# Audio-WestlakeU/NBSS

Measured on AMD Instinct MI355X. Metric: utterances/sec (4 s, 6ch, 129 freqs) SpatialNet bf16 train at 1/2/4/8 MI355X, higher is better.
Workload: dtype bf16; 1 GPU; SpatialNet-small 6ch->2spk, 4-s 8-kHz utterances (32000 samples), n_fft 256/hop 128 (F=129, T=251), 8 layers, full train step (STFT..Adam), bf16 stream + fp32 master/stats, 32 utterances per GPU per step; batch_per_gpu=32, global_batch=32, parallelism=dp1

## Files before the change

### nbss_amd/csrc/full.hip

```cpp
#include <stdlib.h>
#include "launch.h"
#include "layout.h"
#include "prof.h"
#include "blocks.h"
#include "wgrad.h"
#include "fold.h"
#include "foldk.h"
#include "geom.h"
#include "side.h"

#define FL_H 96
#define FL_SQ 8
#define FL_TT_MAX 8
#define FL_KS (FL_H / 32)
#define FL_MT (FL_H / 16)
#define FL_KSF_MAX 5
#define FL_KSF_BIG 9
#define FL_THREADS 512


#define FL_TASK_LOOP_BEGIN(NTASK, WMAT)                                                                                  \
    constexpr bool TPF = TT < 8;                                                                                         \
    Frag<T> anext[KSFM];                                                                                                 \
    if (TPF && w < (NTASK)) {                                                                                            \
        _Pragma("unroll") for (int ks = 0; ks < KSFM; ++ks)                                                              \
            if (ks < ksf) wfrag_load(anext[ks], (WMAT) + (size_t)(w / mtf) * mtf * ksf * 512, w % mtf, ksf, ks);         \
    }                                                                                                                    \
    for (int task = w; task < (NTASK); task += nw) {                                                                     \
        const int ch = task / mtf, mt = task % mtf;                                                                      \
        f32x4 acc = F32X4_ZERO;                                                                                          \
        Frag<T> a[KSFM];                         \
        if (TPF) {                                                                                                       \
            _Pragma("unroll") for (int ks = 0; ks < KSFM; ++ks) a[ks] = anext[ks];                                       \
            const int nx = task + nw;                                                                                    \
            if (nx < (NTASK)) {                                                                                          \
                _Pragma("unroll") for (int ks = 0; ks < KSFM; ++ks)                                                      \
                    if (ks < ksf) wfrag_load(anext[ks], (WMAT) + (size_t)(nx / mtf) * mtf * ksf * 512, nx % mtf, ksf, ks); \
            }                                                                                                            \
        } else {                                                                                                         \
            _Pragma("unroll") for (int ks = 0; ks < KSFM; ++ks)                                                          \
                if (ks < ksf) wfrag_load(a[ks], (WMAT) + (size_t)ch * mtf * ksf * 512, mt, ksf, ks);                     \
        }                                                                                                                \
        _Pragma("unroll") for (int ks = 0; ks < KSFM; ++ks) {                                                            \
            if (ks < ksf) {                                                                                              \
                Frag<T> bq;                                                                                              \
                if (l15 < TT) frag_load(bq, s + ((size_t)ch * TT + l15) * FK + ks * 32 + 8 * g4);                        \
                else frag_zero(bq);                                                                                      \
                acc = mma(a[ks], bq, acc);                                                                               \
            }                                                                                                            \
        }
#define FL_TASK_LOOP_END }

template <class T, int KSFM, int HH, int NSQ, int TT>
__global__ __launch_bounds__(FL_THREADS, HH == 96 && TT == 8 ? 4 : 1)
void full_fwd_kernel(nbss_cfg c, const float* __restrict__ lnw, const float* __restrict__ lnb,
                                                       const float* __restrict__ bs, const float* __restrict__ bfull,
                                                       const float* __restrict__ bu, const T* __restrict__ Wsq,
                                                       const T* __restrict__ Wfull, const T* __restrict__ Wusq,
                                                       const T* __restrict__ x, T* __restrict__ y, int flip) {
    NBSS_LDS(smem);
    const int F = c.F, T_ = c.T;
    const int mtf = cdiv(F, 16), ksf = cdiv(F, 32), FK = ksf * 32, FM = mtf * 16;
    T* s = reinterpret_cast<T*>(smem);
    T* z = s + NSQ * TT * FK;
    const int ntt = cdiv(T_, TT);
    const int bid = flip_bid(flip);
    const int b = bid / ntt, t0 = (bid % ntt) * TT;
    const int tid = threadIdx.x, nthr = blockDim.x;
    const int lane = lane_id(), l15 = lane & 15, g4 = lane >> 4, w = wave_id(), nw = nthr >> 6;
    const int ntile = cdiv(F, 16 / TT);

    for (int i = tid; i < NSQ * TT * FK + FM * TT * NSQ; i += nthr) store1(s + i, 0.f);
    lds_barrier();

    {
        Frag<T> a[(HH / 32)];
#pragma unroll
        for (int ks = 0; ks < (HH / 32); ++ks) wfrag_load(a[ks], Wsq, 0, (HH / 32), ks);
        float gam[(HH / 32)][8], bet[(HH / 32)][8];
#pragma unroll
        for (int ks = 0; ks < (HH / 32); ++ks)
#pragma unroll
            for (int j = 0; j < 8; ++j) {
                gam[ks][j] = lnw[ks * 32 + 8 * g4 + j];
                bet[ks][j] = lnb[ks * 32 + 8 * g4 + j];
            }
        const int tclf = t0 + (l15 % TT) < T_ ? t0 + (l15 % TT) : T_ - 1;
        auto row_of_f = [&](int nt) -> const T* {
            const int f = (16 / TT) * nt + (l15 / TT);
            return x + (((size_t)b * F + (f < F ? f : F - 1)) * T_ + tclf) * HH;
        };
        Frag<T> xnext[(HH / 32)];
        if (w < ntile) {
#pragma unroll
            for (int ks = 0; ks < (HH / 32); ++ks) frag_load(xnext[ks], row_of_f(w) + ks * 32 + 8 * g4);
        }
        for (int nt = w; nt < ntile; nt += nw) {
            const int f = (16 / TT) * nt + (l15 / TT), tt = l15 % TT;
            const bool valid = f < F && t0 + tt < T_;
            Frag<T> xcur[(HH / 32)];
#pragma unroll
            for (int ks = 0; ks < (HH / 32); ++ks) xcur[ks] = xnext[ks];
            {
                const T* nx = row_of_f(nt + nw < ntile ? nt + nw : nt);
#pragma unroll
                for (int ks = 0; ks < (HH / 32); ++ks) frag_load(xnext[ks], nx + ks * 32 + 8 * g4);
            }
            float v[(HH / 32)][8];
            float sum = 0.f;
#pragma unroll
            for (int ks = 0; ks < (HH / 32); ++ks) {
#pragma unroll
                for (int j = 0; j < 8; ++j) {
                    v[ks][j] = keep_if(valid, frag_get(xcur[ks], j));
                    sum += v[ks][j];
                }
            }
            const float mean = wave_sum16(sum) * (1.0f / HH);
            float q = 0.f;
#pragma unroll
            for (int ks = 0; ks < (HH / 32); ++ks)
#pragma unroll
                for (int j = 0; j < 8; ++j) {
                    const float d = v[ks][j] - mean;
                    q += d * d;
                }
            const float rstd = rsqrtf(wave_sum16(q) * (1.0f / HH) + 1e-5f);
            f32x4 acc = F32X4_ZERO;
#pragma unroll
            for (int ks = 0; ks < (HH / 32); ++ks) {
                Frag<T> u;
#pragma unroll
                for (int j = 0; j < 8; ++j) frag_set(u, j, (v[ks][j] - mean) * rstd * gam[ks][j] + bet[ks][j]);
                acc = mma(a[ks], u, acc);
            }
            if (valid && 4 * g4 < NSQ) {
#pragma unroll
                for (int r = 0; r < 4; ++r) {
                    const int ch = 4 * g4 + r;
                    store1(s + ((size_t)ch * TT + tt) * FK + f, silu_f(acc[r] + bs[ch]));
                }
            }
        }
    }
    lds_barrier();

    {
        FL_TASK_LOOP_BEGIN(NSQ * mtf, Wfull)
        if (l15 < TT) {
#pragma unroll
            for (int r = 0; r < 4; ++r) {
                const int k = mt * 16 + 4 * g4 + r;
                if (k < F) store1(z + ((size_t)k * TT + l15) * NSQ + ch, acc[r] + bfull[ch * F + k]);
            }
        }
        FL_TASK_LOOP_END
    }
    lds_barrier();

    {
        Frag<T> a[(HH / 16)];
#pragma unroll
        for (int mt = 0; mt < (HH / 16); ++mt) wfrag_load(a[mt], Wusq, mt, 1, 0);
        const int tcl3 = t0 + (l15 % TT) < T_ ? t0 + (l15 % TT) : T_ - 1;
        auto row_of_3 = [&](int nt) -> const T* {
            const int f = (16 / TT) * nt + (l15 / TT);
            return x + (((size_t)b * F + (f < F ? f : F - 1)) * T_ + tcl3) * HH;
        };
        RawC4<T> rnext[(HH / 16)];
        if (w < ntile) {
#pragma unroll
            for (int mt = 0; mt < (HH / 16); ++mt) rawc_load(rnext[mt], row_of_3(w) + 16 * mt + 4 * g4);
        }
        for (int nt = w; nt < ntile; nt += nw) {
            const int f = (16 / TT) * nt + (l15 / TT), tt = l15 % TT;
            const bool valid = f < F && t0 + tt < T_;
            RawC4<T> rcur[(HH / 16)];
#pragma unroll
            for (int mt = 0; mt < (HH / 16); ++mt) rcur[mt] = rnext[mt];
            {
                const T* nx = row_of_3(nt + nw < ntile ? nt + nw : nt);
#pragma unroll
                for (int mt = 0; mt < (HH / 16); ++mt) rawc_load(rnext[mt], nx + 16 * mt + 4 * g4);
            }
            Frag<T> bq;
            if (8 * g4 < NSQ && f < F) frag_load(bq, z + ((size_t)f * TT + tt) * NSQ + 8 * g4);
            else frag_zero(bq);
            const size_t go = (((size_t)b * F + f) * T_ + t0 + tt) * HH;
#pragma unroll
            for (int mt = 0; mt < (HH / 16); ++mt) {
                f32x4 acc = mma(a[mt], bq, F32X4_ZERO);
                if (valid) {
                    const int ch = 16 * mt + 4 * g4;
                    float xv[4];
                    rawc_get(rcur[mt], xv);
                    float o[4];
#pragma unroll
                    for (int r = 0; r < 4; ++r) o[r] = xv[r] + round_to(silu_f(acc[r] + bu[ch + r]), x);
                    store4(y + go + ch, o[0], o[1], o[2], o[3]);
                }
            }
        }
    }
}

#define FL_FKP(F) (((F) + 3) & ~3)
#define FL_WFR 15

template <class T, int KSFM, int TT>
__global__ __launch_bounds__(FL_THREADS, sizeof(T) == 2 && TT == 8 ? 4 : 2) void full_bwd_kernel(nbss_cfg c, LayerPtrs lp, const float* __restrict__ P, float* __restrict__ part, int layer,
                                                       const T* __restrict__ Wsq, const T* __restrict__ Wfull, const T* __restrict__ Wusq,
                                                       const T* __restrict__ WsqT, const T* __restrict__ WfullT, const T* __restrict__ WusqT,
                                                       const T* __restrict__ x, const T* __restrict__ dy, T* __restrict__ dx,
                                                       float* __restrict__ stats, T* __restrict__ s_out, T* __restrict__ dz_out,
                                                       T* __restrict__ z_out, T* __restrict__ dyp_out, T* __restrict__ dsp_out, int flip) {
    NBSS_LDS(smem);
    const int F = c.F, T_ = c.T;
    const int mtf = cdiv(F, 16), ksf = cdiv(F, 32), FK = ksf * 32, FM = mtf * 16, FKP = FL_FKP(F);
    T* s = reinterpret_cast<T*>(smem);
    T* sp = s + FL_SQ * TT * FK;
    T* z = sp + FM * TT * FL_SQ;
    float* aff = reinterpret_cast<float*>(z + FM * TT * FL_SQ);
    T* wl = reinterpret_cast<T*>(aff + FL_SQ * 17);
    const int ntt = cdiv(T_, TT);
    const int bid = flip_bid(flip);
    const int b = bid / ntt, t0 = (bid % ntt) * TT;
    const int tid = threadIdx.x, nthr = blockDim.x;
    const int lane = lane_id(), l15 = lane & 15, g4 = lane >> 4, w = wave_id(), nw = nthr >> 6;
    const int ntile = cdiv(F, 16 / TT);
    const float* lnw = lp.p[P_FULL_LN_W];
    const float* lnb = lp.p[P_FULL_LN_B];
    const float* bs = lp.p[P_SQ_B];
    const float* bfull = lp.p[P_FULL_B];
    const float* bu = lp.p[P_USQ_B];

    for (int i = tid; i < FL_SQ * TT * FK + 2 * FM * TT * FL_SQ; i += nthr) store1(s + i, 0.f);
    for (int i = tid; i < FL_SQ * 17; i += nthr) aff[i] = 0.f;
    {
        constexpr int VPF = 512 * (int)sizeof(T) / 16;
        for (int v = tid; v < FL_WFR * VPF; v += nthr) {
            const int fr = v / VPF, pc = v % VPF;
            const T* src = fr < 6 ? Wusq + (size_t)fr * 512 : fr < 9 ? WusqT + (size_t)(fr - 6) * 512 : WsqT + (size_t)(fr - 9) * 512;
            reinterpret_cast<u32x4*>(wl)[v] = reinterpret_cast<const u32x4*>(src)[pc];
        }
    }
    PHASE_BEGIN(wl + FL_WFR * 512);
    lds_barrier();
    PHASE(0);

    auto copy_sq_image = [&](T* __restrict__ dst) {
        constexpr int VE = 8 / sizeof(T);
        const int vpr = FKP / VE;
        for (int i = tid; i < FL_SQ * TT * vpr; i += nthr) {
            const int rowi = i / vpr, v = i % vpr, ch = rowi / TT, tt = rowi % TT;
            if (t0 + tt >= T_) continue;
            const u32x2 val = *reinterpret_cast<const u32x2*>(s + ((size_t)ch * TT + tt) * FK + v * VE);
            *reinterpret_cast<u32x2*>(dst + (((size_t)b * T_ + t0 + tt) * FL_SQ + ch) * FKP + v * VE) = val;
        }
    };

    {
        Frag<T> a[FL_KS];
#pragma unroll
        for (int ks = 0; ks < FL_KS; ++ks) wfrag_load(a[ks], Wsq, 0, FL_KS, ks);
        float gam[BK_KS][8], bet[BK_KS][8];
        load_ln_affine(lnw, lnb, gam, bet);
        for (int nt = w; nt < ntile; nt += nw) {
            const int f = (16 / TT) * nt + (l15 / TT), tt = l15 % TT;
            const bool valid = f < F && t0 + tt < T_;
            Frag<T> u[BK_KS];
            ln_strip96<T>(x + (((size_t)b * F + f) * T_ + t0 + tt) * FL_H, valid, gam, bet, u);
            f32x4 acc = F32X4_ZERO;
#pragma unroll
            for (int ks = 0; ks < FL_KS; ++ks) acc = mma(a[ks], u[ks], acc);
            if (valid && g4 < 2) {
                float pre[4];
#pragma unroll
                for (int r = 0; r < 4; ++r) {
                    const int ch = 4 * g4 + r;
                    pre[r] = acc[r] + bs[ch];
                    const float sv = silu_f(pre[r]);
                    store1(s + ((size_t)ch * TT + tt) * FK + f, sv);
                }
                store4(sp + ((size_t)f * TT + tt) * FL_SQ + 4 * g4, pre[0], pre[1], pre[2], pre[3]);
            }
        }
    }
    PHASE(1);
    lds_barrier();
    PHASE(2);
    copy_sq_image(s_out);

    {
        FL_TASK_LOOP_BEGIN(FL_SQ * mtf, Wfull)
        if (l15 < TT) {
#pragma unroll
            for (int r = 0; r < 4; ++r) {
                const int k = mt * 16 + 4 * g4 + r;
                if (k < F) store1(z + ((size_t)k * TT + l15) * FL_SQ + ch, acc[r] + bfull[ch * F + k]);
            }
        }
        FL_TASK_LOOP_END
    }
    PHASE(3);
    lds_barrier();
    PHASE(4);

    {
        const T* wa = wl + (size_t)lane * 8;
        const int tcl = t0 + (l15 % TT) < T_ ? t0 + (l15 % TT) : T_ - 1;
        auto row_of = [&](int nt) -> size_t {
            const int f = (16 / TT) * nt + (l15 / TT);
            return ((size_t)b * F + (f < F ? f : F - 1)) * T_ + tcl;
        };
        constexpr bool PF = true;
        RawC4<T> dnext[BK_MT];
        if (PF && w < ntile) rawc_load_row<T>(dnext, dy + row_of(w) * FL_H);
        for (int nt = w; nt < ntile; nt += nw) {
            const int f = (16 / TT) * nt + (l15 / TT), tt = l15 % TT;
            const bool valid = f < F && t0 + tt < T_;
            const size_t n = ((size_t)b * F + f) * T_ + t0 + tt;
            RawC4<T> dcur[BK_MT];
            if (PF) {
#pragma unroll
                for (int mt = 0; mt < BK_MT; ++mt) dcur[mt] = dnext[mt];
                rawc_load_row<T>(dnext, dy + row_of(nt + nw < ntile ? nt + nw : nt) * FL_H);
            } else {
                rawc_load_row<T>(dcur, dy + row_of(nt) * FL_H);
            }
            Frag<T> bq;
            if (g4 == 0 && f < F) {
                frag_load(bq, z + ((size_t)f * TT + tt) * FL_SQ);
                if (valid) {
                    float zv[8];
                    load8(z + ((size_t)f * TT + tt) * FL_SQ, zv);
                    store4(z_out + n * FL_SQ, zv[0], zv[1], zv[2], zv[3]);
                    store4(z_out + n * FL_SQ + 4, zv[4], zv[5], zv[6], zv[7]);
                }
            } else {
                frag_zero(bq);
            }
            f32x4 dyp[FL_MT];
#pragma unroll
            for (int mt = 0; mt < FL_MT; ++mt) {
                Frag<T> am;
                frag_load(am, wa + mt * 512);
                const f32x4 acc = mma(am, bq, F32X4_ZERO);
                const int ch = 16 * mt + 4 * g4;
                float dv[4];
                rawc_get(dcur[mt], dv);
#pragma unroll
                for (int r = 0; r < 4; ++r) dyp[mt][r] = valid ? dv[r] * dsilu_f(acc[r] + bu[ch + r]) : 0.f;
                if (valid) store4(dyp_out + n * FL_H + ch, dyp[mt][0], dyp[mt][1], dyp[mt][2], dyp[mt][3]);
            }
            f32x4 dzt = F32X4_ZERO;
#pragma unroll
            for (int ks = 0; ks < FL_KS; ++ks) {
                Frag<T> df, atk;
                frag_from_c2(df, dyp[2 * ks], dyp[2 * ks + 1]);
                frag_load(atk, wa + (6 + ks) * 512);
                dzt = mma(atk, df, dzt);
            }
            if (valid && g4 < 2) {
#pragma unroll
                for (int r = 0; r < 4; ++r) {
                    const int ch = 4 * g4 + r;
                    store1(s + ((size_t)ch * TT + tt) * FK + f, dzt[r]);
                }
            }
        }
    }
    PHASE(5);
    lds_barrier();
    PHASE(6);
    copy_sq_image(dz_out);

    {
        FL_TASK_LOOP_BEGIN(FL_SQ * mtf, WfullT)
        float dbs = 0.f;
        if (l15 < TT) {
#pragma unroll
            for (int r = 0; r < 4; ++r) {
                const int h = mt * 16 + 4 * g4 + r;
                if (h < F) {
                    const float pre = load1(sp + ((size_t)h * TT + l15) * FL_SQ + ch);
                    const float v = acc[r] * dsilu_f(pre);
                    dbs += v;
                    store1(z + ((size_t)h * TT + l15) * FL_SQ + ch, v);
                }
            }
        }
        dbs = wave_sum64(dbs);
        if (lane == 0) aff[ch * 17 + mt] = dbs;
        FL_TASK_LOOP_END
    }
    PHASE(7);
    lds_barrier();
    PHASE(8);

    {
        const T* wa = wl + (size_t)(9 * 512) + (size_t)lane * 8;
        const int tcl = t0 + (l15 % TT) < T_ ? t0 + (l15 % TT) : T_ - 1;
        auto row_of = [&](int nt) -> size_t {
            const int f = (16 / TT) * nt + (l15 / TT);
            return ((size_t)b * F + (f < F ? f : F - 1)) * T_ + tcl;
        };
        constexpr bool PF = false;
        RawC4<T> xnext[BK_MT], dnext[BK_MT];
        if (PF && w < ntile) {
            rawc_load_row<T>(xnext, x + row_of(w) * FL_H);
            rawc_load_row<T>(dnext, dy + row_of(w) * FL_H);
        }
        for (int nt = w; nt < ntile; nt += nw) {
            const int f = (16 / TT) * nt + (l15 / TT), tt = l15 % TT;
            const bool valid = f < F && t0 + tt < T_;
            const size_t n = ((size_t)b * F + f) * T_ + t0 + tt;
            RawC4<T> xcur[BK_MT], dcur[BK_MT];
            if (PF) {
#pragma unroll
                for (int mt = 0; mt < BK_MT; ++mt) { xcur[mt] = xnext[mt]; dcur[mt] = dnext[mt]; }
                const size_t nn = row_of(nt + nw < ntile ? nt + nw : nt);
                rawc_load_row<T>(xnext, x + nn * FL_H);
                rawc_load_row<T>(dnext, dy + nn * FL_H);
            } else {
                rawc_load_row<T>(xcur, x + row_of(nt) * FL_H);
                rawc_load_row<T>(dcur, dy + row_of(nt) * FL_H);
            }
            Frag<T> bq;
            if (g4 == 0 && valid) {
                frag_load(bq, z + ((size_t)f * TT + tt) * FL_SQ);
                float dv[8];
                load8(z + ((size_t)f * TT + tt) * FL_SQ, dv);
                store4(dsp_out + n * FL_SQ, dv[0], dv[1], dv[2], dv[3]);
                store4(dsp_out + n * FL_SQ + 4, dv[4], dv[5], dv[6], dv[7]);
            } else {
                frag_zero(bq);
            }
            f32x4 du[BK_MT];
#pragma unroll
            for (int mt = 0; mt < FL_MT; ++mt) {
                Frag<T> am;
                frag_load(am, wa + mt * 512);
                du[mt] = mma(am, bq, F32X4_ZERO);
            }
            ln_bwd_row96_raw_nas<T>(du, xcur, dcur, dx + n * FL_H, stats + n * 2, valid, lnw);
        }
    }
    PHASE(9);
    lds_barrier();
    PHASE(10);
    for (int i = tid; i < FL_SQ; i += nthr) {
        float v = 0.f;
        for (int mt = 0; mt < mtf; ++mt) v += aff[i * 17 + mt];
        part[(size_t)bid * FL_SQ + i] = v;
    }
    PHASE_END();
}
PHASE_READER(nbss_phase_read_full_bwd)

__global__ void full_sq_prep_kernel(float* __restrict__ tmp) {
    for (int i = threadIdx.x; i < FL_SQ * FL_H + FL_SQ + 2 * FL_H; i += blockDim.x) tmp[i] = (i >= FL_SQ * FL_H + FL_SQ && i < FL_SQ * FL_H + FL_SQ + FL_H) ? 1.0f : 0.f;
}
static_assert(FL_H == FK_H && FL_SQ == FK_SQ, "foldk.h");
__global__ void full_sq_finalize_kernel(const float* __restrict__ tmp, const float* __restrict__ Ws, const float* __restrict__ gamma, const float* __restrict__ beta,
                                        float* __restrict__ dWs, float* __restrict__ dbs, float* __restrict__ dgamma, float* __restrict__ dbeta) {
    fk_full_sq_final(tmp, Ws, gamma, beta, dWs, dbs, dgamma, dbeta);
}

static int full_tt(const nbss_cfg& c) {
    static const int forced = [] { const char* e = getenv("NBSS_FULL_TT"); return e ? atoi(e) : 0; }();
    if (forced == 8 || forced == 4 || forced == 2) return forced;
    for (int tt = FL_TT_MAX; tt > 2; tt >>= 1)
        if (c.B * cdiv(c.T, tt) >= 240) return tt;
    return 2;
}

static size_t full_bwd_lds(const nbss_cfg& c, int tt) {
    const size_t esz = c.dtype == NBSS_BF16 ? 2 : 4;
    const int mtf = cdiv(c.F, 16), ksf = cdiv(c.F, 32);
    return ((size_t)FL_SQ * tt * ksf * 32 + (size_t)2 * mtf * 16 * tt * FL_SQ + (size_t)FL_WFR * 512) * esz + FL_SQ * 17 * sizeof(float) + PHASE_LDS_BYTES;
}
static int full_bwd_width(const nbss_cfg& c) {
    int tt = full_tt(c);
    while (tt > 2 && full_bwd_lds(c, tt) > 160 * 1024) tt >>= 1;
    return tt;
}

template <class T, int KSFM, int TT>
static int full_bwd_tt(const nbss_cfg& c, const float* P, float* part, const void* packed, int layer, const void* x, const void* dy, void* dx,
                       float* stats, void* const* o, hipStream_t st) {
    const LayerPtrs lp = layer_ptrs(c, P, layer);
    const int mtf = cdiv(c.F, 16), ksf = cdiv(c.F, 32);
    const size_t lds = full_bwd_lds(c, TT);
    const T* pk = (const T*)packed;
    if (ksf > KSFM || lds > 160 * 1024) return NBSS_EUNSUPPORTED;
    int e = NBSS_SET_MAX_LDS((full_bwd_kernel<T, KSFM, TT>), lds);
    if (e) return e;
    dim3 grid(c.B * cdiv(c.T, TT)), block(FL_THREADS);
    ProfScope ps(PK_FULL_B, st);
    NBSS_LAUNCH((full_bwd_kernel<T, KSFM, TT>), grid, block, lds, st, c, lp, P, part, layer, pk + pack_off(c, layer, K_SQ), pk + pack_off(c, layer, K_FULL),
                pk + pack_off(c, layer, K_USQ), pk + pack_off(c, layer, K_SQ_T), pk + pack_off(c, layer, K_FULL_T), pk + pack_off(c, layer, K_USQ_T),
                (const T*)x, (const T*)dy, (T*)dx, stats, (T*)o[0], (T*)o[1], (T*)o[2], (T*)o[3], (T*)o[4], walk_flip_next());
    return NBSS_CHECK_LAUNCH();
}

template <class T, int KSFM>
static int full_bwd_t(const nbss_cfg& c, const float* P, float* part, const void* packed, int layer, const void* x, const void* dy, void* dx,
                      float* stats, void* const* o, hipStream_t st) {
    switch (full_bwd_width(c)) {
// ... 111 lines not shown
```

### nbss_amd/csrc/wgrad.hip

```cpp
#include "launch.h"
#include "layout.h"
#include "wgrad.h"
#include "fold.h"
#include "foldk.h"
#include <cstdlib>
#include "prof.h"

#define WG_KC 32
#define WG_LD 40
#define WG_TPW 14
#define WG_WAVES 8
#define WG_THREADS (WG_WAVES * 64)

template <class T, int CW>
NBSS_DEV void load_cw(const T* p, float (&v)[8]) {
    if (CW == 8) load8(p, v);
    else load4(p, v);
}

template <class T, int CW, int TPW>
__global__ __launch_bounds__(WG_THREADS, TPW <= 4 ? 4 : 2) void wgrad_kernel(WgradArgs a) {
    NBSS_LDS(smem);
    const int tid = threadIdx.x, lane = lane_id(), l15 = lane & 15, g4 = lane >> 4, w = wave_id();
    const int mg = a.MA / a.groups, ng = a.NB / a.groups;
// ... 152 lines not shown
    }

    if (a.part) {
        const size_t wg = (size_t)blockIdx.y * gridDim.x + blockIdx.x;
        float* pt = a.part + wg * ntot * 256;
        float* pbias = a.part + (size_t)gridDim.y * gridDim.x * ntot * 256 + wg * ntot * 16;
#pragma unroll
        for (int s = 0; s < TPW; ++s) {
            const int tl = s * WG_WAVES + w;
            if (tl < ntot) {
#pragma unroll
                for (int r = 0; r < 4; ++r) pt[((size_t)tl * 4 + r) * 64 + lane] = acc[s][r];
            }
        }
        if (do_bias && tid < rowsA) {
            const int gl = tid / mgp, m = tid % mgp;
            pbias[(size_t)(gl * tpg + (m >> 4) * ntiles) * 16 + (m & 15)] = bsum;
        }
        return;
    }
#pragma unroll
    for (int s = 0; s < TPW; ++s) {
        const int tl = s * WG_WAVES + w;
        if (tl < ntot) {
            const int g = g_lo + tl / tpg, rem = tl % tpg, mt = rem / ntiles, nt = rem % ntiles;
            const int q = (nt0 + nt) * 16 + l15;
            if (q < nexp) {
                const int tap = q / ng, i = q % ng;
#pragma unroll
                for (int r = 0; r < 4; ++r) {
                    const int m = mt * 16 + 4 * g4 + r;
                    if (m < mv && i < nv) atomicAdd(a.dW + ((size_t)(g * mv + m) * nv + i) * a.taps + tap, acc[s][r]);
                }
            }
        }
    }
    if (do_bias && tid < rowsA) {
        const int g = g_lo + tid / mgp, m = tid % mgp;
        if (m < mv) atomicAdd(a.dbias + (size_t)g * mv + m, bsum);
    }
}


NBSS_HD int tr_ld(int cols) {
    int ld = cols + 16;
    while (ld % 32 != 16) ld += 8;
    return ld;
}

#ifdef NBSS_PHASE_PROF
#define WG_PROBE(bit) (a.dbg & (bit))
#define WG_PROBE_HOST(args, bit) ((args).dbg & (bit))
#else
#define WG_PROBE(bit) false
#define WG_PROBE_HOST(args, bit) false
#endif
#define W3_MAXV 7
#define W3_BS 3

template <int W3_KC, int NS>
__global__ __launch_bounds__(WG_THREADS, NS > 14 ? 1 : 2) void wgrad_tr3_kernel(WgradArgs a) {
    constexpr int NBUF = 2;
    NBSS_LDS(smem);
    typedef bf16_t T;
    const int tid = threadIdx.x, lane = lane_id(), l15 = lane & 15, g4 = lane >> 4, w = wave_id_u();
    const int mg = a.MA / a.groups, ng = a.NB / a.groups;
    const int mv = a.mvalid ? a.mvalid : mg, nv = a.nvalid ? a.nvalid : ng;
    const int mtiles = cdiv(mg, 16), nexp = a.taps * ng, ntiles = cdiv(nexp, 16);
    const bool per_group = gridDim.y > 1;
    const int g_lo = per_group ? blockIdx.y : 0, ngrp = per_group ? 1 : a.groups;
    const int acols0 = g_lo * mg, ncolsA = ngrp * mg, bcols0 = g_lo * ng, ncolsB = ngrp * ng;
    const int lda = tr_ld(ncolsA), ldb = tr_ld(ncolsB);
    const bool fmode = a.taps > 1 && a.shift_dim == 1;
    const int rs = fmode ? 2 : 1;
    const int h = a.taps / 2, rowsB = W3_KC + 2 * h * rs;
    const int imgA = W3_KC * lda, img = imgA + rowsB * ldb;
    T* base = reinterpret_cast<T*>(smem);
    for (int i = tid; i < NBUF * img / 2; i += WG_THREADS) reinterpret_cast<uint32_t*>(base)[i] = 0u;
    float* lnp = reinterpret_cast<float*>(base + (size_t)NBUF * img);
    if (a.stats)
        for (int i = tid; i < 2 * a.NB; i += WG_THREADS) lnp[i] = i < a.NB ? a.gamma[i] : a.beta[i - a.NB];

    f32x4 acc[NS], bacc[W3_BS];
#pragma unroll
    for (int s = 0; s < NS; ++s) acc[s] = F32X4_ZERO;
#pragma unroll
    for (int s = 0; s < W3_BS; ++s) bacc[s] = F32X4_ZERO;
    Frag<T> ones;
#pragma unroll
    for (int jq = 0; jq < 8; ++jq) frag_set(ones, jq, 1.0f);
    const bool do_bias = a.dbias != nullptr;
    const T* Ag = reinterpret_cast<const T*>(a.A);
    const T* Bg = reinterpret_cast<const T*>(a.B);
    const int pA = ncolsA / 8, pB = ncolsB / 8;
    const int nvA = W3_KC * pA, nvec = nvA + rowsB * pB;
    const int nfirst = ngrp * mtiles, ntot = nfirst * ntiles;

    constexpr bool GW = NS > 14;
    int oa[GW ? 3 : NS], ob[GW ? 9 : NS];
    const int trow = 4 * g4 + (l15 >> 2), tcol = 4 * (l15 & 3);
    if constexpr (GW) {
#pragma unroll
        for (int mt = 0; mt < 3; ++mt) oa[mt] = trow * lda + w * mg + mt * 16 + tcol;
#pragma unroll
        for (int nt = 0; nt < 9; ++nt) {
            const int q0 = nt * 16 + tcol;
            ob[nt] = imgA + ((q0 / ng) * rs + trow) * ldb + w * ng + q0 % ng;
        }
    } else {
#pragma unroll
        for (int s = 0; s < NS; ++s) {
            const int tl = s * WG_WAVES + w;
            oa[s] = trow * lda + tcol; ob[s] = imgA + trow * ldb + tcol;
            if (tl < ntot) {
                const int nt = tl / nfirst, gm = tl % nfirst, g = gm / mtiles, mt = gm % mtiles;
                oa[s] = trow * lda + g * mg + mt * 16 + tcol;
                int q0 = nt * 16 + tcol;
                if (q0 >= nexp) q0 = 0;
                ob[s] = imgA + ((q0 / ng) * rs + trow) * ldb + g * ng + q0 % ng;
            }
        }
    }
    const int rsA = a.a_gw ? a.a_gw : a.lda, rsB = a.b_gw ? a.b_gw : a.ldb;
    const int UA = cdiv(nvA, WG_THREADS);
    int vkk[W3_MAXV], vtok[W3_MAXV], vdst[W3_MAXV];
    unsigned vgo[W3_MAXV];
    bool vt1[W3_MAXV], vok[W3_MAXV];
    const int tokB0 = fmode ? -h * a.T : -h;
#pragma unroll
    for (int u = 0; u < W3_MAXV; ++u) {
        const bool isA = u < UA;
        const int v = tid + (isA ? u : u - UA) * WG_THREADS;
        vok[u] = isA ? v < nvA : v < nvec - nvA;
        const int pp = isA ? pA : pB, r = vok[u] ? v / pp : 0, c8 = vok[u] ? v % pp : 0;
        const int col = (isA ? acols0 : bcols0) + 8 * c8, gw = isA ? a.a_gw : a.b_gw, gs = isA ? a.a_gs : a.b_gs, rsg = isA ? rsA : rsB;
        const int hh = isA ? 0 : h;
        vkk[u] = fmode ? r / 2 - hh : r - hh;
        vt1[u] = fmode && (r & 1);
        vtok[u] = fmode ? (r / 2 - hh) * a.T + (r & 1) : r - hh;
        vgo[u] = (unsigned)((vtok[u] - (isA ? 0 : tokB0)) * rsg + (gw ? (col / gw) * gs + col % gw : col));
        vdst[u] = (isA ? 0 : imgA) + r * (isA ? lda : ldb) + 8 * c8;
    }
    const int cpr = cdiv(a.T, W3_KC);
    const int nfc = cdiv(a.F, W3_KC / 2), ntp = cdiv(a.T, 2);
    const int nchunks = fmode ? (a.Ntok / (a.F * a.T)) * ntp * nfc : a.taps > 1 ? (a.Ntok / a.T) * cpr : cdiv(a.Ntok, W3_KC);
    const int r0 = fmode ? nfc : a.taps > 1 ? cpr : 1, r1 = fmode ? ntp : 1;
    const int G = gridDim.x, d0 = G % r0, d1 = (G / r0) % r1, d2 = G / r0 / r1;
    int c0 = (int)blockIdx.x % r0, c1 = ((int)blockIdx.x / r0) % r1, c2 = (int)blockIdx.x / r0 / r1;
    u32x4 pre[W3_MAXV];
    float pmu[W3_MAXV], prs[W3_MAXV];
    auto prefetch = [&]() {
        long nbase;
        int lo, span;
        bool t1ok = true;
        if (fmode) {
            const int t0 = 2 * c1, f0 = c0 * (W3_KC / 2);
            nbase = ((long)c2 * a.F + f0) * a.T + t0; lo = -f0; span = a.F; t1ok = t0 + 1 < a.T;
        } else if (a.taps > 1) {
            const int t0 = c0 * W3_KC;
            nbase = ((long)c2 * r1 + c1) * a.T + t0; lo = -t0; span = a.T;
        } else {
            nbase = ((long)c2 * r1 + c1) * W3_KC; lo = 0; span = a.Ntok - (int)nbase;
        }
        c0 += d0; c1 += d1; c2 += d2;
        if (c0 >= r0) { c0 -= r0; ++c1; }
        if (c1 >= r1) { c1 -= r1; ++c2; }
        const T* Ab = Ag + nbase * rsA;
        const T* Bb = Bg + (nbase + tokB0) * rsB;
        const float* sb = a.stats ? a.stats + 2 * nbase : nullptr;
#pragma unroll
        for (int u = 0; u < W3_MAXV; ++u) {
            pre[u] = (u32x4){0, 0, 0, 0};
            pmu[u] = 0.f; prs[u] = 0.f;
            if (!vok[u] || (unsigned)(vkk[u] - lo) >= (unsigned)span || (vt1[u] && !t1ok) || WG_PROBE(4)) continue;
            const T* sbase = u < UA ? Ab : Bb;
            pre[u] = *reinterpret_cast<const u32x4*>(reinterpret_cast<const char*>(sbase) + (size_t)(vgo[u] * 2u));
            if (!GW && u >= UA && sb) { pmu[u] = sb[2 * vtok[u]]; prs[u] = sb[2 * vtok[u] + 1]; }
        }
    };
    auto stash = [&](T* buf) {
#pragma unroll
        for (int u = 0; u < W3_MAXV; ++u) {
            if (!vok[u] || WG_PROBE(8)) continue;
            u32x4 x = pre[u];
            if (!GW && u >= UA && a.stats) {
                float f[8];
#pragma unroll
                for (int i = 0; i < 4; ++i) { f[2 * i] = bf2f((bf16_t)(x[i] & 0xFFFF)); f[2 * i + 1] = bf2f((bf16_t)(x[i] >> 16)); }
                float gm[8], bt[8];
                const int col = (int)vgo[u] - (vtok[u] - tokB0) * rsB;
                load8(lnp + col, gm);
                load8(lnp + a.NB + col, bt);
#pragma unroll
                for (int e = 0; e < 8; ++e) f[e] = prs[u] != 0.f ? (f[e] - pmu[u]) * prs[u] * gm[e] + bt[e] : 0.f;
#pragma unroll
                for (int i = 0; i < 4; ++i) x[i] = pack2bf(f[2 * i], f[2 * i + 1]);
            }
            *reinterpret_cast<u32x4*>(buf + vdst[u]) = x;
        }
    };

    int ch = blockIdx.x;
    if (WG_PROBE(16)) return;
    if (ch < nchunks) prefetch();
    lds_barrier();
    int b = 0;
    for (; ch < nchunks; ch += gridDim.x) {
        T* buf = base + (size_t)b * img;
        stash(buf);
        lds_barrier();
        if (ch + (int)gridDim.x < nchunks) prefetch();
        constexpr int KH = W3_KC / 32;
        Frag<T> fa[2], fb[2];
        if (WG_PROBE(2)) { b ^= 1; continue; }
        if constexpr (GW) {
            Frag<T> ga[3];
#pragma unroll
            for (int mt = 0; mt < 3; ++mt) {
                frag_load_tr(ga[mt], buf + oa[mt], lda);
                bacc[mt] = mma(ga[mt], ones, bacc[mt]);
            }
            frag_load_tr(fb[0], buf + ob[0], ldb);
#pragma unroll
            for (int nt = 0; nt < 9; ++nt) {
                if (nt + 1 < 9) frag_load_tr(fb[(nt + 1) & 1], buf + ob[nt + 1], ldb);
#pragma unroll
                for (int mt = 0; mt < 3; ++mt) acc[nt * 3 + mt] = mma(ga[mt], fb[nt & 1], acc[nt * 3 + mt]);
            }
        } else {
        frag_load_tr(fa[0], buf + oa[0], lda);
        frag_load_tr(fb[0], buf + ob[0], ldb);
#pragma unroll
        for (int i = 0; i < NS * KH; ++i) {
            const int s = i / KH, cur = i & 1;
            if (i + 1 < NS * KH) {
                const int s1 = (i + 1) / KH, kh1 = (i + 1) % KH;
                frag_load_tr(fa[cur ^ 1], buf + oa[s1] + kh1 * 32 * lda, lda);
                frag_load_tr(fb[cur ^ 1], buf + ob[s1] + kh1 * 32 * ldb, ldb);
            }
            acc[s] = mma(fa[cur], fb[cur], acc[s]);
            if (s < W3_BS) bacc[s < W3_BS ? s : 0] = mma(fa[cur], ones, bacc[s < W3_BS ? s : 0]);
        }
        }
        if (NBUF == 1) lds_barrier();
        else b ^= 1;
    }

    if (WG_PROBE(1)) return;
    if (a.part) {
        const size_t wg = (size_t)blockIdx.y * gridDim.x + blockIdx.x;
        float* pt = a.part + wg * ntot * 256;
        float* pbias = a.part + (size_t)gridDim.y * gridDim.x * ntot * 256 + wg * ntot * 16;
        if constexpr (GW) {
#pragma unroll
            for (int nt = 0; nt < 9; ++nt)
#pragma unroll
                for (int mt = 0; mt < 3; ++mt) {
                    const int tl = nt * nfirst + w * 3 + mt;
#pragma unroll
                    for (int r = 0; r < 4; ++r) pt[((size_t)tl * 4 + r) * 64 + lane] = acc[nt * 3 + mt][r];
                }
            if (do_bias && l15 == 0) {
#pragma unroll
                for (int mt = 0; mt < 3; ++mt)
#pragma unroll
                    for (int r = 0; r < 4; ++r) pbias[(w * 3 + mt) * 16 + 4 * g4 + r] = bacc[mt][r];
            }
            return;
        }
#pragma unroll
        for (int s = 0; s < NS; ++s) {
            const int tl = s * WG_WAVES + w;
            if (tl < ntot) {
#pragma unroll
                for (int r = 0; r < 4; ++r) pt[((size_t)tl * 4 + r) * 64 + lane] = acc[s][r];
                if (s < W3_BS && do_bias && tl < nfirst && l15 == 0) {
#pragma unroll
                    for (int r = 0; r < 4; ++r) pbias[tl * 16 + 4 * g4 + r] = bacc[s < W3_BS ? s : 0][r];
                }
            }
        }
        return;
    }
#pragma unroll
    for (int s = 0; s < NS; ++s) {
        const int tl = s * WG_WAVES + w;
        if (tl < ntot) {
            const int nt = tl / nfirst, gm = tl % nfirst, g = g_lo + gm / mtiles, mt = gm % mtiles;
            const int q = nt * 16 + l15;
            if (q < nexp) {
                const int tap = q / ng, i = q % ng;
#pragma unroll
                for (int r = 0; r < 4; ++r) {
                    const int m = mt * 16 + 4 * g4 + r;
                    if (m < mv && i < nv) atomicAdd(a.dW + ((size_t)(g * mv + m) * nv + i) * a.taps + tap, acc[s][r]);
                }
            }
            if (s < W3_BS && do_bias && nt == 0 && l15 == 0) {
#pragma unroll
                for (int r = 0; r < 4; ++r) {
                    const int m = mt * 16 + 4 * g4 + r;
                    if (m < mv) atomicAdd(a.dbias + (size_t)g * mv + m, bacc[s < W3_BS ? s : 0][r]);
                }
            }
        }
    }
}


#define WG_RSL 4
static_assert(WG_RSL == FK_RSL, "foldk.h");
__global__ __launch_bounds__(64 * WG_RSL) void wgrad_reduce_kernel(WgradArgs a, int xb, int nt_major) {
    NBSS_LDS(smem);
    fk_wgrad_reduce(a, xb, nt_major, (int)blockIdx.x, (int)blockIdx.z, (int)gridDim.z, reinterpret_cast<float*>(smem));
}

static int wgrad_reduce_go(const WgradArgs& a, int ntot, int xb, int ybl, int nt_major, hipStream_t st, bool batched = false) {
    if (batched && g_fold) {
        g_fold->st = st;
        FoldItem it;
        it.kind = FK_WGRAD_REDUCE;
        it.gx = 4 * ntot; it.gy = ybl; it.nblk = it.gx * it.gy;
        it.u.wr.a = a; it.u.wr.xb = xb; it.u.wr.nt_major = nt_major;
        return g_fold->add(1, it);
    }
    NBSS_FOLD_LAUNCH(wgrad_reduce_kernel, dim3(4 * ntot, 1, ybl), dim3(64 * WG_RSL), WG_RSL * 80 * sizeof(float), st, a, xb, nt_major);
    return NBSS_CHECK_LAUNCH();
}
static int fold_part(WgradArgs& a, size_t need, bool* batched) {
    *batched = false;
    if (!g_fold || !a.part) return NBSS_OK;
    int err;
    void* p = g_fold->alloc(need, &err);
    if (err) return err;
    if (!p) return g_fold->flush();
    a.part = (float*)p;
    *batched = true;
    return NBSS_OK;
}

int wgrad_reduce_launch(const WgradArgs& a, int ntot, int xb, hipStream_t st) { return wgrad_reduce_go(a, ntot, xb, 1, 1, st); }

template <class T>
static int wgrad_launch_t(const WgradArgs& a_in, hipStream_t st) {
    const WgradArgs& a = a_in;
    const int mg = a.MA / a.groups, ng = a.NB / a.groups;
    const int mtiles = cdiv(mg, 16), ntiles = cdiv(a.taps * ng, 16), tpg = mtiles * ntiles;
    const int cap = WG_WAVES * WG_TPW;
    int nz = 1;
    if (tpg > cap) {
        if (a.taps != 1 || mtiles > cap) return NBSS_EUNSUPPORTED;
        nz = cdiv(ntiles, cap / mtiles);
        nz = cdiv(ntiles, cdiv(ntiles, nz));
    }
    const int ntz = cdiv(ntiles, nz);
    size_t lds_all = (size_t)a.groups * (mtiles + ntiles) * 16 * WG_LD * sizeof(T);
    const bool all = nz == 1 && a.groups * tpg <= cap && lds_all <= 80 * 1024 && mtiles * 16 * a.groups <= WG_THREADS;
    const int ybl = all ? 1 : a.groups;
    const size_t lds = all ? lds_all : (size_t)(mtiles + ntz) * 16 * WG_LD * sizeof(T);
    if (lds > 160 * 1024 || mtiles * 16 > WG_THREADS) return NBSS_EUNSUPPORTED;
    const bool cw8 = mg % 8 == 0 && ng % 8 == 0 && a.lda % 8 == 0 && a.ldb % 8 == 0 && sizeof(T) == 2;
    const int nchunks = cdiv(a.Ntok, WG_KC);
    const int ncA = all ? a.MA : mg, ncB = all ? a.NB : ng;
    if (sizeof(T) == 2 && !all && nz == 1 && a.taps > 1 && a.shift_dim == 0 && a.shift_stride == 1 && a.Ntok % a.T == 0 && a.groups * tpg <= WG_WAVES * 27 &&
        a.groups == WG_WAVES && mtiles == 3 && ntiles == 9 && a.taps * ng == 144 && a.MA % 8 == 0 && a.NB % 8 == 0 && a.lda % 8 == 0 && a.ldb % 8 == 0 && !a.a_gw && !a.b_gw && !a.stats && a.part && !WG_PROBE_HOST(a, 1)) {
        const int kc = 32, h3 = a.taps / 2, rowsB = kc + 2 * h3;
        const size_t img = ((size_t)kc * tr_ld(a.MA) + (size_t)rowsB * tr_ld(a.NB)) * 2;
        const int nvec = (cdiv(kc * (a.MA / 8), WG_THREADS) + cdiv(rowsB * (a.NB / 8), WG_THREADS)) * WG_THREADS;
        const size_t lds3 = 2 * img + 2 * (size_t)a.NB * sizeof(float);
        const int ntot3 = a.groups * tpg;
        int xb = 256;
        const int nch = (a.Ntok / a.T) * cdiv(a.T, kc);
        if (xb > nch) xb = nch;
        if (nvec <= W3_MAXV * WG_THREADS && lds3 <= 158 * 1024 && (size_t)xb * ntot3 * 272 * sizeof(float) <= WGPART_BYTES) {
            ProfScope ps(PK_WGRAD, st);
            int e3;
            WgradArgs a27 = a;
            bool batched;
            if ((e3 = fold_part(a27, (size_t)xb * ntot3 * 272 * sizeof(float), &batched))) return e3;
            if ((e3 = NBSS_SET_MAX_LDS((wgrad_tr3_kernel<32, 27>), lds3))) return e3;
            NBSS_LAUNCH((wgrad_tr3_kernel<32, 27>), dim3(xb, 1), dim3(WG_THREADS), lds3, st, a27);
            if ((e3 = NBSS_CHECK_LAUNCH())) return e3;
            return wgrad_reduce_go(a27, ntot3, xb, 1, 1, st, batched);
        }
    }
    if (nz == 1 && sizeof(T) == 2 && ncA % 8 == 0 && ncB % 8 == 0 && a.lda % 8 == 0 && a.ldb % 8 == 0) {
        const bool fmode3 = a.taps > 1 && a.shift_dim == 1 && a.shift_stride == a.T && a.Ntok % (a.F * a.T) == 0;
        const bool tmode3 = a.taps > 1 && a.shift_dim == 0 && a.shift_stride == 1 && a.Ntok % a.T == 0;
        const bool skinny = a.taps == 1 && cdiv((all ? a.groups : 1) * mtiles * ntiles, WG_WAVES) <= 2;
        const int kc3 = fmode3 ? 96 : skinny ? 128 : 64, h3 = a.taps / 2, rowsB3 = kc3 + 2 * h3 * (fmode3 ? 2 : 1), nfirst3 = (all ? a.groups : 1) * mtiles;
        const size_t img3 = ((size_t)kc3 * tr_ld(ncA) + (size_t)rowsB3 * tr_ld(ncB)) * 2;
        const int nvec3 = (cdiv(kc3 * (ncA / 8), WG_THREADS) + cdiv(rowsB3 * (ncB / 8), WG_THREADS)) * WG_THREADS;
        const bool gm_ok = (!a.a_gw || a.a_gw % 8 == 0) && (!a.b_gw || (a.b_gw % 8 == 0 && !a.stats));
        if (gm_ok && (a.taps == 1 || tmode3 || fmode3) && nvec3 <= W3_MAXV * WG_THREADS && nfirst3 <= WG_WAVES * W3_BS &&
            2 * img3 + 2 * (size_t)a.NB * sizeof(float) <= 158 * 1024) {
            const int nch3 = fmode3 ? (a.Ntok / (a.F * a.T)) * cdiv(a.T, 2) * cdiv(a.F, kc3 / 2) : tmode3 ? (a.Ntok / a.T) * cdiv(a.T, kc3) : cdiv(a.Ntok, kc3);
            int xb = 256 / ybl;
            if (xb < 16) xb = 16;
            if (xb > nch3) xb = nch3;
            ProfScope ps(PK_WGRAD, st);
            const size_t lds3 = 2 * img3 + 2 * (size_t)a.NB * sizeof(float);
            const int ntot3 = nfirst3 * ntiles;
            WgradArgs a3 = a;
            if ((size_t)ybl * xb * ntot3 * 272 * sizeof(float) > WGPART_BYTES) a3.part = nullptr;
            int e3;
            bool batched;
            if ((e3 = fold_part(a3, (size_t)ybl * xb * ntot3 * 272 * sizeof(float), &batched))) return e3;
            const int need = cdiv(ntot3, WG_WAVES);
#define W3_GO(KC, NS)                                                                             \
    do {                                                                                          \
        if ((e3 = NBSS_SET_MAX_LDS((wgrad_tr3_kernel<KC, NS>), lds3))) return e3;                 \
        NBSS_LAUNCH((wgrad_tr3_kernel<KC, NS>), dim3(xb, ybl), dim3(WG_THREADS), lds3, st, a3);   \
    } while (0)
            if (fmode3) {
                if (need <= 5) W3_GO(96, 5);
                else W3_GO(96, 14);
            } else if (skinny) W3_GO(128, 2);
            else if (need <= 2) W3_GO(64, 2);
            else if (need <= 5) W3_GO(64, 5);
            else if (need <= 10) W3_GO(64, 10);
            else W3_GO(64, 14);
#undef W3_GO
            if ((e3 = NBSS_CHECK_LAUNCH())) return e3;
            if (a3.part && !WG_PROBE_HOST(a3, 1)) {
                return wgrad_reduce_go(a3, ntot3, xb, ybl, 1, st, batched);
            }
            return NBSS_OK;
        }
    }
    if (a.a_gw || a.b_gw) return NBSS_EUNSUPPORTED;
    const bool small = (all ? a.groups : 1) * mtiles * ntz <= WG_WAVES * 4 && sizeof(T) == 2;
    int xbl = (small ? 1024 : 384) / (ybl * nz);
    if (xbl < 16) xbl = 16;
    if (xbl > nchunks) xbl = nchunks;
    dim3 grid(xbl, ybl, nz), block(WG_THREADS);
    ProfScope ps(PK_WGRAD, st);
    int e;
    WgradArgs ak = a_in;
    const int ntot_k = (all ? a.groups : 1) * tpg;
    if (nz > 1 || (size_t)ybl * xbl * ntot_k * 272 * sizeof(float) > WGPART_BYTES) ak.part = nullptr;
    bool batched;
    if ((e = fold_part(ak, (size_t)ybl * xbl * ntot_k * 272 * sizeof(float), &batched))) return e;
#define WK_GO(CW, TPW)                                                             \
    do {                                                                           \
        if ((e = NBSS_SET_MAX_LDS((wgrad_kernel<T, CW, TPW>), lds))) return e;     \
        NBSS_LAUNCH((wgrad_kernel<T, CW, TPW>), grid, block, lds, st, ak);         \
    } while (0)
    if (cw8 && small) WK_GO(8, 4);
    else if (cw8) WK_GO(8, WG_TPW);
    else if (small) WK_GO(4, 4);
    else WK_GO(4, WG_TPW);
#undef WK_GO
    if ((e = NBSS_CHECK_LAUNCH())) return e;
    if (ak.part) {
        return wgrad_reduce_go(ak, ntot_k, xbl, ybl, 0, st, batched);
    }
    return NBSS_OK;
}

int wgrad_launch(const WgradArgs& a0, int dtype, hipStream_t st) {
    WgradArgs a = a0;
#ifdef NBSS_PHASE_PROF
    static const int dbg = getenv("NBSS_WG_DEBUG") ? atoi(getenv("NBSS_WG_DEBUG")) : 0;
    a.dbg = dbg;
#endif
    if (a.MA % a.groups || a.NB % a.groups) return NBSS_EINVAL;
    const int mg = a.MA / a.groups, ng = a.NB / a.groups;
    if (mg % 4 || ng % 4) return NBSS_EUNSUPPORTED;
    return dtype == NBSS_BF16 ? wgrad_launch_t<bf16_t>(a, st) : wgrad_launch_t<float>(a, st);
}
```

Baseline: 739.7 utterances/s.

## Add multi-stage LDS ring weight-gradient kernel using direct global-to-LDS DMA

Adds a new weight-gradient GEMM kernel that streams K-chunks of both operands into a 3- or 4-deep LDS ring buffer using global_load_lds_dwordx4, with partial waitcnt so loads for later chunks overlap the MFMA work on the current one. It is selected for single-tap, stats-free cases that have a partial buffer, and its outputs go to the existing reduce kernel. Separately, the padded F stride in the fused backward kernel is rounded to a multiple of 8 instead of 4. The ring uses more LDS and depends on hand-written waitcnt encoding and inline asm that manipulates m0, so a wrong count or occupancy loss is possible.

```diff
diff --git a/nbss_amd/csrc/full.hip b/nbss_amd/csrc/full.hip
--- a/nbss_amd/csrc/full.hip
+++ b/nbss_amd/csrc/full.hip
@@ -204,7 +204,7 @@
     }
 }
 
-#define FL_FKP(F) (((F) + 3) & ~3)
+#define FL_FKP(F) (((F) + 7) & ~7)
 #define FL_WFR 15
 
 template <class T, int KSFM, int TT>
diff --git a/nbss_amd/csrc/wgrad.hip b/nbss_amd/csrc/wgrad.hip
--- a/nbss_amd/csrc/wgrad.hip
+++ b/nbss_amd/csrc/wgrad.hip
@@ -478,6 +478,165 @@
                     const int m = mt * 16 + 4 * g4 + r;
                     if (m < mv) atomicAdd(a.dbias + (size_t)g * mv + m, bacc[s < W3_BS ? s : 0][r]);
                 }
+            }
+        }
+    }
+}
+
+
+#define W3R_MAXQ 6
+#ifndef W3R_DMAX
+#define W3R_DMAX 4
+#endif
+#define W3R_LDS (156 * 1024)
+static_assert(W3R_MAXQ * (W3R_DMAX - 2) <= 12, "w3r_wait");
+
+NBSS_DEV void w3r_wait(int n) {
+#ifndef NBSS_EMU
+#define W3R_W(N) case N: __builtin_amdgcn_s_waitcnt(0x0F70 | (N & 15) | ((N >> 4) << 14)); break;
+    switch (n) {
+        W3R_W(1) W3R_W(2) W3R_W(3) W3R_W(4) W3R_W(5) W3R_W(6) W3R_W(7) W3R_W(8) W3R_W(9) W3R_W(10) W3R_W(11) W3R_W(12)
+        default: __builtin_amdgcn_s_waitcnt(0x0F70); break;
+    }
+#undef W3R_W
+#endif
+}
+
+NBSS_DEV void w3r_dma16(void* lds_wave_base, const void* g) {
+#ifdef NBSS_EMU
+    dma16_to_lds(lds_wave_base, g);
+#else
+    unsigned keep;
+    const unsigned dst = (unsigned)(size_t)lds_wave_base;
+    asm volatile("s_mov_b32 %0, m0\n\ts_mov_b32 m0, %2\n\ts_nop 0\n\tglobal_load_lds_dwordx4 %1, off\n\ts_mov_b32 m0, %0"
+                 : "=&s"(keep) : "v"(g), "s"(dst) : "memory");
+#endif
+}
+
+template <int KC, int NS, int D>
+__global__ __launch_bounds__(WG_THREADS, 2) void wgrad_ring_kernel(WgradArgs a) {
+    NBSS_LDS(smem);
+    typedef bf16_t T;
+    const int tid = threadIdx.x, lane = lane_id(), l15 = lane & 15, g4 = lane >> 4, w = wave_id_u();
+    const int mg = a.MA / a.groups, ng = a.NB / a.groups;
+    const int mtiles = cdiv(mg, 16), ntiles = cdiv(ng, 16);
+    const bool per_group = gridDim.y > 1;
+    const int g_lo = per_group ? blockIdx.y : 0, ngrp = per_group ? 1 : a.groups;
+    const int acols0 = g_lo * mg, ncolsA = ngrp * mg, bcols0 = g_lo * ng, ncolsB = ngrp * ng;
+    const int lda = tr_ld(ncolsA), ldb = tr_ld(ncolsB);
+    const int imgA = KC * lda, img = imgA + KC * ldb;
+    T* base = reinterpret_cast<T*>(smem);
+    for (int i = tid; i < D * img / 2; i += WG_THREADS) reinterpret_cast<uint32_t*>(base)[i] = 0u;
+
+    f32x4 acc[NS], bacc[W3_BS];
+#pragma unroll
+    for (int s = 0; s < NS; ++s) acc[s] = F32X4_ZERO;
+#pragma unroll
+    for (int s = 0; s < W3_BS; ++s) bacc[s] = F32X4_ZERO;
+    Frag<T> ones;
+#pragma unroll
+    for (int jq = 0; jq < 8; ++jq) frag_set(ones, jq, 1.0f);
+    const bool do_bias = a.dbias != nullptr;
+    const T* Ag = reinterpret_cast<const T*>(a.A);
+    const T* Bg = reinterpret_cast<const T*>(a.B);
+    const int nfirst = ngrp * mtiles, ntot = nfirst * ntiles;
+
+    int oa[NS], ob[NS];
+    const int trow = 4 * g4 + (l15 >> 2), tcol = 4 * (l15 & 3);
+#pragma unroll
+    for (int s = 0; s < NS; ++s) {
+        const int tl = s * WG_WAVES + w;
+        oa[s] = trow * lda + tcol; ob[s] = imgA + trow * ldb + tcol;
+        if (tl < ntot) {
+            const int nt = tl / nfirst, gm = tl % nfirst, g = gm / mtiles, mt = gm % mtiles;
+            oa[s] = trow * lda + g * mg + mt * 16 + tcol;
+            int q0 = nt * 16 + tcol;
+            if (q0 >= ng) q0 = 0;
+            ob[s] = imgA + trow * ldb + g * ng + q0;
+        }
+    }
+    const int rsA = a.a_gw ? a.a_gw : a.lda, rsB = a.b_gw ? a.b_gw : a.ldb;
+    const int npA = imgA / 8, pla = lda / 8, plb = ldb / 8, pA = ncolsA / 8, pB = ncolsB / 8;
+    const int npc = img / 8 - (plb - pB);
+    const int ninstr = cdiv(npc, 64);
+    int vrow[W3R_MAXQ];
+    unsigned vgo[W3R_MAXQ];
+#pragma unroll
+    for (int q = 0; q < W3R_MAXQ; ++q) {
+        const int p = (w + WG_WAVES * q) * 64 + lane;
+        vrow[q] = -1; vgo[q] = 0u;
+        if (p < npc) {
+            const bool isA = p < npA;
+            const int pp = isA ? p : p - npA, pl = isA ? pla : plb, r = pp / pl, c8 = pp % pl;
+            vrow[q] = KC;
+            if (c8 < (isA ? pA : pB)) {
+                const int col = (isA ? acols0 : bcols0) + 8 * c8, gw = isA ? a.a_gw : a.b_gw, gs = isA ? a.a_gs : a.b_gs;
+                vrow[q] = r;
+                vgo[q] = (unsigned)(r * (isA ? rsA : rsB) + (gw ? (col / gw) * gs + col % gw : col));
+            }
+        }
+    }
+    const int nq = w < ninstr ? (ninstr - 1 - w) / WG_WAVES + 1 : 0;
+    const int nchunks = cdiv(a.Ntok, KC), G = gridDim.x;
+    const int mine = (int)blockIdx.x < nchunks ? (nchunks - 1 - (int)blockIdx.x) / G + 1 : 0;
+    auto issue = [&](int i) {
+        const long nbase = ((long)blockIdx.x + (long)i * G) * KC;
+        const int span = a.Ntok - nbase < KC ? (int)(a.Ntok - nbase) : KC;
+        const char* Ab = reinterpret_cast<const char*>(Ag + nbase * rsA);
+        const char* Bb = reinterpret_cast<const char*>(Bg + nbase * rsB);
+        char* sb = reinterpret_cast<char*>(base + (size_t)(i % D) * img);
+#pragma unroll
+        for (int q = 0; q < W3R_MAXQ; ++q) {
+            const int j = w + WG_WAVES * q;
+            if (j >= ninstr || WG_PROBE(4)) continue;
+            const char* sbase = j * 64 < npA ? Ab : Bb;
+            if ((unsigned)vrow[q] < (unsigned)span) w3r_dma16(sb + j * 1024, sbase + (size_t)(vgo[q] * 2u));
+            else if (span < KC && vrow[q] >= 0) *reinterpret_cast<u32x4*>(sb + j * 1024 + lane * 16) = (u32x4){0, 0, 0, 0};
+        }
+    };
+
+    if (WG_PROBE(16)) return;
+    lds_barrier();
+#pragma unroll
+    for (int i = 0; i < D - 1; ++i)
+        if (i < mine) issue(i);
+    for (int i = 0; i < mine; ++i) {
+        if (i + D - 2 <= mine - 2) w3r_wait(nq * (D - 2));
+        else dma_wait_all();
+        lds_barrier();
+        if (i + D - 1 < mine) issue(i + D - 1);
+        if (WG_PROBE(2)) continue;
+        const T* buf = base + (size_t)(i % D) * img;
+        constexpr int KH = KC / 32;
+        Frag<T> fa[2], fb[2];
+        frag_load_tr(fa[0], buf + oa[0], lda);
+        frag_load_tr(fb[0], buf + ob[0], ldb);
+#pragma unroll
+        for (int k = 0; k < NS * KH; ++k) {
+            const int s = k / KH, cur = k & 1;
+            if (k + 1 < NS * KH) {
+                const int s1 = (k + 1) / KH, kh1 = (k + 1) % KH;
+                frag_load_tr(fa[cur ^ 1], buf + oa[s1] + kh1 * 32 * lda, lda);
+                frag_load_tr(fb[cur ^ 1], buf + ob[s1] + kh1 * 32 * ldb, ldb);
+            }
+            acc[s] = mma(fa[cur], fb[cur], acc[s]);
+            if (s < W3_BS) bacc[s < W3_BS ? s : 0] = mma(fa[cur], ones, bacc[s < W3_BS ? s : 0]);
+        }
+    }
+
+    if (WG_PROBE(1)) return;
+    const size_t wg = (size_t)blockIdx.y * gridDim.x + blockIdx.x;
+    float* pt = a.part + wg * ntot * 256;
+    float* pbias = a.part + (size_t)gridDim.y * gridDim.x * ntot * 256 + wg * ntot * 16;
+#pragma unroll
+    for (int s = 0; s < NS; ++s) {
+        const int tl = s * WG_WAVES + w;
+        if (tl < ntot) {
+#pragma unroll
+            for (int r = 0; r < 4; ++r) pt[((size_t)tl * 4 + r) * 64 + lane] = acc[s][r];
+            if (s < W3_BS && do_bias && tl < nfirst && l15 == 0) {
+#pragma unroll
+                for (int r = 0; r < 4; ++r) pbias[tl * 16 + 4 * g4 + r] = bacc[s < W3_BS ? s : 0][r];
             }
         }
     }
@@ -583,6 +742,30 @@
             bool batched;
             if ((e3 = fold_part(a3, (size_t)ybl * xb * ntot3 * 272 * sizeof(float), &batched))) return e3;
             const int need = cdiv(ntot3, WG_WAVES);
+            const size_t stage3 = img3;
+            const int depth = a.taps == 1 && !a.stats && a3.part && !WG_PROBE_HOST(a3, 32) && cdiv((int)(stage3 / 1024), WG_WAVES) <= W3R_MAXQ
+                                  ? (W3R_DMAX * stage3 <= W3R_LDS ? W3R_DMAX : 3 * stage3 <= W3R_LDS ? 3 : 0) : 0;
+#define W3R_GO(KC, NS)                                                                                          \
+    do {                                                                                                        \
+        if (depth == 3) {                                                                                       \
+            if ((e3 = NBSS_SET_MAX_LDS((wgrad_ring_kernel<KC, NS, 3>), 3 * stage3))) return e3;                 \
+            NBSS_LAUNCH((wgrad_ring_kernel<KC, NS, 3>), dim3(xb, ybl), dim3(WG_THREADS), 3 * stage3, st, a3);   \
+        } else {                                                                                                \
+            if ((e3 = NBSS_SET_MAX_LDS((wgrad_ring_kernel<KC, NS, W3R_DMAX>), W3R_DMAX * stage3))) return e3;   \
+            NBSS_LAUNCH((wgrad_ring_kernel<KC, NS, W3R_DMAX>), dim3(xb, ybl), dim3(WG_THREADS), W3R_DMAX * stage3, st, a3); \
+        }                                                                                                       \
+    } while (0)
+            if (depth) {
+                if (skinny) W3R_GO(128, 2);
+                else if (need <= 2) W3R_GO(64, 2);
+                else if (need <= 5) W3R_GO(64, 5);
+                else if (need <= 10) W3R_GO(64, 10);
+                else W3R_GO(64, 14);
+                if ((e3 = NBSS_CHECK_LAUNCH())) return e3;
+                if (WG_PROBE_HOST(a3, 1)) return NBSS_OK;
+                return wgrad_reduce_go(a3, ntot3, xb, ybl, 1, st, batched);
+            }
+#undef W3R_GO
 #define W3_GO(KC, NS)                                                                             \
     do {                                                                                          \
         if ((e3 = NBSS_SET_MAX_LDS((wgrad_tr3_kernel<KC, NS>), lds3))) return e3;                 \
```

Result: no change. 746.9 utterances/s, median of 6 (+1.0%).
